# uibk-uncover/ws-unet

Hardware: AMD Instinct MI355X
Metric: 512x512 grayscale images/sec (UNet predict) (higher is better)
Workload: dtype f16 MFMA on the f16 halves + ONE block-scaled fp4 (e2m1) MFMA per tap pair for both residual cross terms (per-pixel / per-(co, tap) E8M0 scales), fp32 accumulate; planar storage

## Files before the change

### ws_unet_amd/csrc/conv3x3_q.hip

```cpp
#include "wsu_device.h"
#include <cstdlib>

#ifndef WSU_Q_EPO
#define WSU_Q_EPO 1
#endif
#ifndef WSU_Q_PIPE2
#define WSU_Q_PIPE2 0
#endif
#ifndef WSU_Q_PIPE_DEPTH
#define WSU_Q_PIPE_DEPTH 1
#endif
#ifndef WSU_Q_PROBE_NOX8
#define WSU_Q_PROBE_NOX8 0
#endif
#ifndef WSU_Q_EPO_FENCE
#define WSU_Q_EPO_FENCE 1
#endif

namespace {

constexpr int TW = 32, TH = 16, IW = TW + 2, IH = TH + 2;
constexpr int NPIX = IW * IH;
constexpr int PLANE = NPIX * 16;
constexpr int IN_SEG = (NPIX + 63) / 64;
constexpr int S_LDS = IN_SEG * 256;
constexpr int IN_SLOT = 3 * PLANE + S_LDS;
constexpr int W_GRAN = 9 * 3 * WSU_COB * 16;
constexpr int W_SLOT = W_GRAN + 1024;
constexpr int NIN = 3, NWS = 2;
constexpr int W_BASE = NIN * IN_SLOT;
constexpr int LDS_EXTRA = W_BASE + NWS * W_SLOT;
constexpr int LDS_TOTAL = LDS_EXTRA + 1024 * 4 + 4 * 64 * 4 + 16;
static_assert(LDS_TOTAL <= 160 * 1024 && W_SLOT % 1024 == 0, "LDS budget");
constexpr int NLOAD = 4;
constexpr int W_PIECES = W_SLOT / 1024;
constexpr unsigned OOB = 0xFFFFFFF0u;
constexpr int IN_SLOT_H = 2 * PLANE;
constexpr int W_SLOT_H = 9 * 2 * WSU_COB * 16;
template <int FMT> struct QGeo {
    static_assert(FMT == WSU_PLANAR_Q || FMT == WSU_PLANAR_H, "conv3x3_q_kernel formats: Q and H");
    static constexpr bool H = FMT == WSU_PLANAR_H;
    static constexpr int in_slot = H ? IN_SLOT_H : IN_SLOT, w_slot = H ? W_SLOT_H : W_SLOT;
    static constexpr int w_planes = H ? 2 : 3;
    static constexpr int w_base = NIN * in_slot, lds_extra = w_base + NWS * w_slot;
    static constexpr int lds_total = lds_extra + 1024 * 4 + 4 * 64 * 4 + 16;
    static constexpr int w_pieces = w_slot / 1024;
};
static_assert(QGeo<WSU_PLANAR_Q>::lds_total == LDS_TOTAL && QGeo<WSU_PLANAR_Q>::w_pieces == W_PIECES && W_SLOT_H % 1024 == 0, "LDS geometry");

struct QArgs {
    const char* x1; const char* x2; const char* wp; const float* bias;
    char* y; char* ypool;
    const float* head_w; const float* head_b; float* head_out; float* head_logit; int head_cout;
    int n, h, w, c1, c2, cout;
    int tiles_x, tiles_y, ncb, nch1, nch;
    int relu;
    int ntiles;
    unsigned* range_flag;
    int msplit;
    int ablate;
    const float* img; const float* w1; const float* b1;
};

struct Tile { int n, y0, x0, cb, mh; };
__device__ __forceinline__ Tile tile_of(const QArgs& a, int t) {
    Tile r;
    r.cb = t % a.ncb; t /= a.ncb;
    const int tx = t % a.tiles_x; t /= a.tiles_x;
    const int ty = t % a.tiles_y;
    r.n = t / a.tiles_y; r.y0 = ty * TH; r.x0 = tx * TW;
    r.mh = 0;
    if (a.msplit) { r.mh = r.cb & 1; r.cb >>= 1; }
    return r;
}

typedef __attribute__((address_space(3))) void lds_void;
typedef __attribute__((address_space(3))) char lds_char;

__device__ __forceinline__ float dpp_xor1(float v) {
    return __builtin_bit_cast(float, __builtin_amdgcn_update_dpp(0, __builtin_bit_cast(int, v), 0xB1 , 0xF, 0xF, true));
}

template <int FMT, int LW>
__device__ __forceinline__ void q_loader(const QArgs& a, char* smem, int lane, int lw, int G, int J) {
    using Gm = QGeo<FMT>;
    constexpr int NSEG = LW < 2 ? 3 : 2;
    constexpr int NIN_OPS = (Gm::H ? 2 : 4) * NSEG;
    constexpr int W0 = Gm::H ? (LW < 2 ? LW * 3 : 6 + (LW - 2) * 6) : (LW < 2 ? LW * 5 : 10 + (LW - 2) * 9);
    constexpr int NWP = Gm::H ? (LW < 2 ? 3 : 6) : (LW < 2 ? 5 : 9);
    static_assert(2 * 5 + 2 * 9 == W_PIECES && 2 * 3 + 2 * 6 == QGeo<WSU_PLANAR_H>::w_pieces, "weight pieces over the loader waves");
    lds_char* smem3 = (lds_char*)smem;
    const unsigned hw16 = (unsigned)(a.h * a.w) * 16u;
    const unsigned chunk_bytes = Gm::H ? (unsigned)wsu_h_chunk_bytes(a.h, a.w) : (unsigned)wsu_q_chunk_bytes(a.h, a.w);
    unsigned voff[NSEG], soff[NSEG];
    auto plan = [&](const Tile& t) __attribute__((always_inline)) {
        WSU_STATIC_FOR(NSEG, k, {
            const int idx = min((LW + NLOAD * k) * 64 + lane, NPIX - 1);
            const int r = idx / IW, c = idx - r * IW;
            const int yy = wsu_reflect(t.y0 - 1 + r, a.h), xx = wsu_reflect(t.x0 - 1 + c, a.w);
            voff[k] = (unsigned)(yy * a.w + xx) * 16u;
            if constexpr (!Gm::H) soff[k] = 3u * hw16 + wsu_q_soff(yy, xx, a.tiles_x);
        });
    };
    Tile ti = tile_of(a, lw); int ci = 0, kti = 0;
    int cbw = ti.cb, cw = 0, ktw = 0;
    auto issue_in = [&](int s) __attribute__((always_inline)) {
        const char* in_src = ci < a.nch1 ? a.x1 + ((size_t)ti.n * a.nch1 + ci) * chunk_bytes : a.x2 + ((size_t)ti.n * (a.nch - a.nch1) + (ci - a.nch1)) * chunk_bytes;
        const auto rs_in = __builtin_amdgcn_make_buffer_rsrc(const_cast<char*>(in_src), 0, (int)chunk_bytes, 0x00020000);
        lds_char* slot = smem3 + (s % NIN) * Gm::in_slot;
        WSU_STATIC_FOR(NSEG, k, {
            constexpr int seg = LW + NLOAD * k;
            const bool live = seg < IN_SEG - 1 || lane < NPIX - (IN_SEG - 1) * 64;
            if (live) {
                __builtin_amdgcn_raw_ptr_buffer_load_lds(rs_in, (lds_void*)(slot + seg * 1024), 16, voff[k], 0, 0, 0);
                __builtin_amdgcn_raw_ptr_buffer_load_lds(rs_in, (lds_void*)(slot + PLANE + seg * 1024), 16, voff[k], (int)hw16, 0, 0);
                if constexpr (!Gm::H) {
                    __builtin_amdgcn_raw_ptr_buffer_load_lds(rs_in, (lds_void*)(slot + 2 * PLANE + seg * 1024), 16, voff[k], (int)(2u * hw16), 0, 0);
                    __builtin_amdgcn_raw_ptr_buffer_load_lds(rs_in, (lds_void*)(slot + 3 * PLANE + seg * 256), 1, soff[k], 0, 0, 0);
                }
            }
        });
        if (++ci == a.nch && s + 1 < J) { ci = 0; ++kti; ti = tile_of(a, lw + kti * G); plan(ti); }
    };
    auto issue_w = [&](int s) __attribute__((always_inline)) {
        const auto rs_w = __builtin_amdgcn_make_buffer_rsrc(const_cast<char*>(a.wp), 0, 0x7FFFFFF0, 0x00020000);
        const int w_base = (cbw * a.nch + cw) * Gm::w_slot;
        lds_char* slot = smem3 + Gm::w_base + (s % NWS) * Gm::w_slot;
        WSU_STATIC_FOR(NWP, k, {
            constexpr int piece = W0 + k;
            __builtin_amdgcn_raw_ptr_buffer_load_lds(rs_w, (lds_void*)(slot + piece * 1024), 16, (unsigned)lane * 16u, w_base + piece * 1024, 0, 0);
        });
        if (++cw == a.nch && s + 1 < J) { cw = 0; ++ktw; cbw = tile_of(a, lw + ktw * G).cb; }
    };
    if (J <= 0) return;
    plan(ti);
    issue_w(0);
    issue_in(0);
    if (J > 1) issue_in(1);
    if (J > 1) asm volatile("s_waitcnt vmcnt(%0)" :: "n"(NIN_OPS) : "memory"); else asm volatile("s_waitcnt vmcnt(0)" ::: "memory");
    for (int j = 0; ; ++j) {
        __builtin_amdgcn_s_barrier();
        asm volatile("" ::: "memory");
        if (j + 1 >= J) break;
        if (!(a.ablate & 1)) {
            issue_w(j + 1);
            const bool more = j + 2 < J;
            if (more) issue_in(j + 2);
            if (more) asm volatile("s_waitcnt vmcnt(%0)" :: "n"(NIN_OPS) : "memory"); else asm volatile("s_waitcnt vmcnt(0)" ::: "memory");
        }
    }
}

__device__ __forceinline__ void q_loader_f1(const QArgs& a, char* smem, int lane, int lw, int G, int J, int lw8) {
    if (J <= 0) return;
    if (a.ablate & 16) __builtin_amdgcn_s_setprio(3);
    lds_char* smem3 = (lds_char*)smem;
    constexpr int F1_PX = 3;
    float pimg[F1_PX][9];
    float f1_max = 0.f;
    Tile ti = tile_of(a, lw); int ci = 0, kti = 0;
    int cbw = ti.cb, cw = 0, ktw = 0;
    auto window = [&](const Tile& tt) __attribute__((always_inline)) {
        const float* img = a.img + (size_t)tt.n * a.h * a.w;
#pragma unroll
        for (int k = 0; k < F1_PX; ++k) {
            const int idx = min((lw8 + NLOAD * k) * 64 + lane, NPIX - 1);
            const int r = idx / IW, cc = idx - r * IW;
            const int yy = wsu_reflect(tt.y0 - 1 + r, a.h), xx = wsu_reflect(tt.x0 - 1 + cc, a.w);
#pragma unroll
            for (int tp = 0; tp < 9; ++tp)
                pimg[k][tp] = img[(size_t)wsu_reflect(yy + tp / 3 - 1, a.h) * a.w + wsu_reflect(xx + tp % 3 - 1, a.w)];
        }
    };
    typedef __attribute__((address_space(4))) const f32x2 cst_f32x2;
    auto compute_in = [&](int s) __attribute__((always_inline)) {
        char* slot = smem + (s % NIN) * IN_SLOT;
        cst_f32x2* wt = (cst_f32x2*)(a.w1 + ci * 16);
        cst_f32x2* bt = (cst_f32x2*)(a.b1 + ci * 16);
        f32x2 acc[F1_PX][8];
#pragma unroll
        for (int g = 0; g < 8; ++g) {
            const f32x2 b = bt[g];
#pragma unroll
            for (int k = 0; k < F1_PX; ++k) acc[k][g] = b;
        }
#pragma unroll
        for (int tp = 0; tp < 9; ++tp) {
            f32x2 wv[8];
#pragma unroll
            for (int g = 0; g < 8; ++g) wv[g] = wt[tp * 32 + g];
#pragma unroll
            for (int k = 0; k < F1_PX; ++k) {
                const f32x2 pw = {pimg[k][tp & ~1], pimg[k][(tp | 1) < 9 ? (tp | 1) : tp]};
#pragma unroll
                for (int g = 0; g < 8; ++g) {
                    if (tp & 1) asm volatile("v_pk_fma_f32 %0, %1, %2, %0 op_sel:[1,0,0] op_sel_hi:[1,1,1]" : "+v"(acc[k][g]) : "v"(pw), "s"(wv[g]));
                    else asm volatile("v_pk_fma_f32 %0, %1, %2, %0 op_sel:[0,0,0] op_sel_hi:[0,1,1]" : "+v"(acc[k][g]) : "v"(pw), "s"(wv[g]));
                }
            }
        }
        asm volatile("s_nop 0" ::: "memory");
#pragma unroll
        for (int k = 0; k < F1_PX; ++k) {
            const int idx = (lw8 + NLOAD * k) * 64 + lane;
            f32x4 v[4];
#pragma unroll
            for (int g = 0; g < 4; ++g) v[g] = mk_f4(acc[k][2 * g][0], acc[k][2 * g][1], acc[k][2 * g + 1][0], acc[k][2 * g + 1][1]);
#pragma unroll
            for (int g = 0; g < 4; ++g)
#pragma unroll
                for (int e = 0; e < 4; ++e) { v[g][e] = fmaxf(v[g][e], 0.f); f1_max = fmaxf(f1_max, v[g][e]); }
            u32x4 h0, h1, qg; uint32_t sb;
            wsu_q4_encode16(v, h0, h1, qg, sb);
            if (lw8 + NLOAD * k < IN_SEG && idx < NPIX) {
                char* d = slot + idx * 16;
                *reinterpret_cast<u32x4*>(d) = h0;
                *reinterpret_cast<u32x4*>(d + PLANE) = h1;
                *reinterpret_cast<u32x4*>(d + 2 * PLANE) = qg;
                *reinterpret_cast<uint32_t*>(slot + 3 * PLANE + idx * 4) = sb;
            }
        }
        if (++ci == a.nch && s + 1 < J) { ci = 0; ++kti; ti = tile_of(a, lw + kti * G); window(ti); }
    };
    const int w0 = lw8 < 2 ? lw8 * 5 : 10 + (lw8 - 2) * 9, nwp = lw8 < 2 ? 5 : 9;
    auto issue_w = [&](int s) __attribute__((always_inline)) {
        const auto rs_w = __builtin_amdgcn_make_buffer_rsrc(const_cast<char*>(a.wp), 0, 0x7FFFFFF0, 0x00020000);
        const int w_base = (cbw * a.nch + cw) * W_SLOT;
        lds_char* slot = smem3 + W_BASE + (s % NWS) * W_SLOT;
#pragma unroll
        for (int k = 0; k < 9; ++k)
            if (k < nwp)
                __builtin_amdgcn_raw_ptr_buffer_load_lds(rs_w, (lds_void*)(slot + (w0 + k) * 1024), 16, (unsigned)lane * 16u, w_base + (w0 + k) * 1024, 0, 0);
        if (++cw == a.nch && s + 1 < J) { cw = 0; ++ktw; cbw = tile_of(a, lw + ktw * G).cb; }
    };
    window(ti);
    issue_w(0);
    compute_in(0);
    if (J > 1) compute_in(1);
    asm volatile("s_waitcnt vmcnt(0) lgkmcnt(0)" ::: "memory");
    for (int j = 0; ; ++j) {
        __builtin_amdgcn_s_barrier();
        asm volatile("" ::: "memory");
        if (j + 1 >= J) break;
        issue_w(j + 1);
        if (j + 2 < J) compute_in(j + 2);
        asm volatile("s_waitcnt vmcnt(0) lgkmcnt(0)" ::: "memory");
    }
    if (a.range_flag && __builtin_amdgcn_ballot_w64(!(f1_max <= WSU_F8_RANGE)) != 0 && lane == 0) atomicOr(a.range_flag, 1u);
}

template <int RQ, int HC, bool POOL, bool FQ, bool MSPLIT, bool F1 = false, int FMT = WSU_PLANAR_Q>
__global__ __launch_bounds__((16 / RQ + NLOAD) * 64) __attribute__((amdgpu_waves_per_eu(RQ == 4 ? 2 : 3, RQ == 4 ? 2 : 3)))
void conv3x3_q_kernel(const QArgs a) {
    using Gm = QGeo<FMT>;
    constexpr bool H = Gm::H;
    static_assert(!(H && F1), "the fused first layer computes Q inputs");
    constexpr int NWAVE = 16 / RQ, NT = (NWAVE + NLOAD) * 64;
    extern __shared__ __attribute__((aligned(16))) char smem[];
    const int tid = threadIdx.x;
    const int wv = __builtin_amdgcn_readfirstlane(tid >> 6), lane = tid & 63, l31 = lane & 31, hh = lane >> 5;
    const int l31_k = l31, hh_k = hh;
    const int G = gridDim.x;
    const int lw = (int)wsu_xcd_remap(blockIdx.x, G);
    const int K = a.ntiles > lw ? (a.ntiles - lw + G - 1) / G : 0;
    const int J = K * a.nch;

    float* s_bias = reinterpret_cast<float*>(smem + Gm::lds_extra);
    float* s_hw = s_bias + 1024;
    float* s_hb = s_hw + 4 * 64;
    for (int i = tid; i < a.cout; i += NT) s_bias[i] = a.bias ? a.bias[i] : 0.f;
    constexpr bool HEAD = HC > 0;
    if constexpr (HEAD) {
        for (int i = tid; i < a.head_cout * 64; i += NT) s_hw[i] = a.head_w[i];
        if (tid < 4) s_hb[tid] = (a.head_b && tid < a.head_cout) ? a.head_b[tid] : 0.f;
    }

    if (wv >= NWAVE) {
        if constexpr (F1) { q_loader_f1(a, smem, lane, lw, G, J, wv - NWAVE); return; }
        switch (wv - NWAVE) {
            case 0: q_loader<FMT, 0>(a, smem, lane, lw, G, J); break;
            case 1: q_loader<FMT, 1>(a, smem, lane, lw, G, J); break;
            case 2: q_loader<FMT, 2>(a, smem, lane, lw, G, J); break;
            default: q_loader<FMT, 3>(a, smem, lane, lw, G, J); break;
        }
        return;
    }

    Tile cur = tile_of(a, lw);
    constexpr int MH = MSPLIT ? 1 : 2;
    constexpr bool PIPE = (RQ == 4 || WSU_Q_PIPE2) && !H;
    constexpr bool EPO = WSU_Q_EPO && !MSPLIT && HC == 0 && RQ != 4;
    f32x16 acc[2][4];
    int kt = 0, j = 0;
    unsigned q_in_off = 0, q_w_off = 0;
    const char* ldsA = smem;
    const char* ldsB = smem;
    int hh_q = hh;
    auto begin_step = [&]() __attribute__((always_inline)) {
        __builtin_amdgcn_s_barrier();
        asm volatile("" ::: "memory");
        q_in_off = (unsigned)(j % NIN) * Gm::in_slot; q_w_off = Gm::w_base + (unsigned)(j % NWS) * Gm::w_slot;
        ldsA = smem + q_w_off + (cur.mh * 32 + l31) * 16;
        ldsB = smem + q_in_off + ((RQ * wv) * IW + l31) * 16;
        hh_q = hh;
        asm volatile("" : "+v"(hh_q));
    };
    auto zero_acc = [&]() __attribute__((always_inline)) {
#pragma unroll
        for (int m = 0; m < MH; ++m)
#pragma unroll
            for (int q = 0; q < RQ; ++q)
#pragma unroll
                for (int r = 0; r < 16; ++r) acc[m][q][r] = 0.f;
    };
    auto main_term = [&](auto tap_c, auto ms_c) __attribute__((always_inline)) {
        constexpr int tap = decltype(tap_c)::value, dy = tap / 3, dx = tap % 3;
        constexpr int ms = decltype(ms_c)::value, ML = ms < 0 ? 0 : ms, MU = ms < 0 ? MH : ms + 1;
        u32x4 ah[2], bh[4];
_Pragma("unroll")
        for (int m = ML; m < MU; ++m) ah[m] = *reinterpret_cast<const u32x4*>(ldsA + ((tap * Gm::w_planes + hh) * 64 + m * 32) * 16);
_Pragma("unroll")
        for (int q = 0; q < RQ; ++q) bh[q] = *reinterpret_cast<const u32x4*>(ldsB + hh * PLANE + ((q + dy) * IW + dx) * 16);
_Pragma("unroll")
        for (int m = ML; m < MU; ++m)
_Pragma("unroll")
            for (int q = 0; q < RQ; ++q) wsu_mfma_f16(ah[m], bh[q], acc[m][q]);
    };
    auto cross_q4 = [&](auto tp_c, auto ms_c) __attribute__((always_inline)) {
        constexpr int tp = decltype(tp_c)::value;
        constexpr int ms = decltype(ms_c)::value, ML = ms < 0 ? 0 : ms, MU = ms < 0 ? MH : ms + 1;
        constexpr int t0 = 2 * tp, t1 = (2 * tp + 1 < 9) ? 2 * tp + 1 : 2 * tp;
        constexpr bool single = 2 * tp + 1 >= 9;
        const int tap = hh_q ? t1 : t0;
        const int pixoff = (tap / 3) * IW + tap % 3;
        u32x4 a4[2], b4[4]; int sa[2], sb[4];
        typedef __attribute__((address_space(3))) const unsigned char lds_cuchar;
        typedef __attribute__((address_space(3))) const int lds_cint;
        typedef __attribute__((address_space(3))) const u32x4 lds_cu32x4;
        lds_char* L = (lds_char*)smem;
        const unsigned wbase = q_w_off + (unsigned)(cur.mh * 32 + l31) * 16u + (unsigned)((tap * 3 + 2) * 64) * 16u;
        const unsigned sabase = q_w_off + W_GRAN + (unsigned)(tap * 64 + cur.mh * 32 + l31);
        const unsigned pix = (unsigned)((RQ * wv) * IW + l31 + pixoff);
_Pragma("unroll")
        for (int m = ML; m < MU; ++m) {
            a4[m] = *(lds_cu32x4*)(L + wbase + m * 32 * 16);
            sa[m] = *(lds_cuchar*)(L + sabase + m * 32);
        }
_Pragma("unroll")
        for (int q = 0; q < RQ; ++q) {
            b4[q] = *(lds_cu32x4*)(L + q_in_off + 2 * PLANE + (pix + q * IW) * 16u);
            sb[q] = *(lds_cint*)(L + q_in_off + 3 * PLANE + (pix + q * IW) * 4u);
        }
        if (single && hh_q) {
            const u32x4 z = mk_u4(0, 0, 0, 0);
_Pragma("unroll")
            for (int m = ML; m < MU; ++m) a4[m] = z;
_Pragma("unroll")
            for (int q = 0; q < RQ; ++q) b4[q] = z;
        }
_Pragma("unroll")
        for (int m = ML; m < MU; ++m)
_Pragma("unroll")
            for (int q = 0; q < RQ; ++q) wsu_mfma_q4(a4[m], b4[q], sa[m], sb[q], acc[m][q]);
    };
    auto units_range = [&](auto ms_c, auto lo_c, auto hi_c) __attribute__((always_inline)) {
        constexpr int lo = decltype(lo_c)::value, hi = decltype(hi_c)::value;
        if constexpr (EPO) asm volatile("" : "+v"(hh_q));
        WSU_STATIC_FOR(hi - lo, i, {
            constexpr int tp = lo + i;
            if constexpr (!H && !(WSU_Q_PROBE_NOX8 && tp == 4)) cross_q4(std::integral_constant<int, tp>{}, ms_c);
            main_term(std::integral_constant<int, 2 * tp>{}, ms_c);
            if constexpr (2 * tp + 1 < 9) main_term(std::integral_constant<int, 2 * tp + 1>{}, ms_c);
        });
    };
    constexpr std::integral_constant<int, -1> all_m{};
    struct Frag { u32x4 a[2]; u32x4 b[4]; int sa[2]; int sb[4]; };
    auto load_unit = [&](auto u_c, Frag& f) __attribute__((always_inline)) {
        constexpr int u = decltype(u_c)::value, tp = u / 3, k = u % 3;
        typedef __attribute__((address_space(3))) const unsigned char lds_cuchar;
        typedef __attribute__((address_space(3))) const int lds_cint;
        typedef __attribute__((address_space(3))) const u32x4 lds_cu32x4;
        lds_char* L = (lds_char*)smem;
        if constexpr (k == 0) {
            constexpr int t0 = 2 * tp, t1 = (2 * tp + 1 < 9) ? 2 * tp + 1 : 2 * tp;
            const int tap = hh_q ? t1 : t0;
            const int pixoff = (tap / 3) * IW + tap % 3;
            const unsigned wbase = q_w_off + (unsigned)(cur.mh * 32 + l31) * 16u + (unsigned)((tap * 3 + 2) * 64) * 16u;
            const unsigned sabase = q_w_off + W_GRAN + (unsigned)(tap * 64 + cur.mh * 32 + l31);
            const unsigned pix = (unsigned)((RQ * wv) * IW + l31 + pixoff);
_Pragma("unroll")
            for (int m = 0; m < MH; ++m) {
                f.a[m] = *(lds_cu32x4*)(L + wbase + m * 32 * 16);
                f.sa[m] = *(lds_cuchar*)(L + sabase + m * 32);
            }
_Pragma("unroll")
            for (int q = 0; q < RQ; ++q) {
                f.b[q] = *(lds_cu32x4*)(L + q_in_off + 2 * PLANE + (pix + q * IW) * 16u);
                f.sb[q] = *(lds_cint*)(L + q_in_off + 3 * PLANE + (pix + q * IW) * 4u);
            }
        } else {
            constexpr int tap = 2 * tp + k - 1, dy = tap / 3, dx = tap % 3;
            const unsigned abase = q_w_off + (unsigned)((cur.mh * 32 + l31) * 16) + (unsigned)(hh_q * 64 * 16);
            const unsigned bbase = q_in_off + (unsigned)(((RQ * wv) * IW + l31) * 16) + (unsigned)(hh_q * PLANE);
_Pragma("unroll")
            for (int m = 0; m < MH; ++m) f.a[m] = *(lds_cu32x4*)(L + abase + ((tap * 3) * 64 + m * 32) * 16);
_Pragma("unroll")
            for (int q = 0; q < RQ; ++q) f.b[q] = *(lds_cu32x4*)(L + bbase + ((q + dy) * IW + dx) * 16);
        }
    };
    auto mma_unit = [&](auto u_c, Frag& f) __attribute__((always_inline)) {
        constexpr int u = decltype(u_c)::value, tp = u / 3, k = u % 3;
        if constexpr (k == 0) {
            if (2 * tp + 1 >= 9 && hh_q) {
                const u32x4 z = mk_u4(0, 0, 0, 0);
_Pragma("unroll")
                for (int m = 0; m < MH; ++m) f.a[m] = z;
_Pragma("unroll")
                for (int q = 0; q < RQ; ++q) f.b[q] = z;
            }
_Pragma("unroll")
            for (int m = 0; m < MH; ++m)
_Pragma("unroll")
                for (int q = 0; q < RQ; ++q) wsu_mfma_q4(f.a[m], f.b[q], f.sa[m], f.sb[q], acc[m][q]);
        } else {
_Pragma("unroll")
            for (int m = 0; m < MH; ++m)
_Pragma("unroll")
                for (int q = 0; q < RQ; ++q) wsu_mfma_f16(f.a[m], f.b[q], acc[m][q]);
        }
    };
    auto units_pipelined = [&]() __attribute__((always_inline)) {
        constexpr int NU = 14, D = WSU_Q_PIPE_DEPTH, NS = D + 1;
        Frag fr[NS];
        WSU_STATIC_FOR(D, u, { load_unit(u_c, fr[u % NS]); });
        WSU_STATIC_FOR(NU, u, {
            if constexpr (u + D < NU) load_unit(std::integral_constant<int, u + D>{}, fr[(u + D) % NS]);
            __builtin_amdgcn_sched_barrier(0);
            mma_unit(u_c, fr[u % NS]);
            __builtin_amdgcn_sched_barrier(0);
        });
    };
    auto units_all = [&](auto ms_c) __attribute__((always_inline)) {
        if constexpr (PIPE && decltype(ms_c)::value < 0) { units_pipelined(); return; }
        units_range(ms_c, std::integral_constant<int, 0>{}, std::integral_constant<int, 5>{});
    };

    auto finish_tile = [&]() __attribute__((always_inline)) {
        int l31 = l31_k, hh = hh_k;
        asm volatile("" : "+v"(l31), "+v"(hh));
        const int col = cur.x0 + l31;
        const unsigned hw16 = (unsigned)(a.h * a.w) * 16u;
        const int nco = a.cout >> 4;
        float hz[4][HC > 0 ? HC : 1];
        float vmax = 0.f;
        const float relu_floor = a.relu ? 0.f : -__builtin_inff();
#pragma unroll
        for (int q = 0; q < RQ; ++q)
#pragma unroll
            for (int o = 0; o < (HC > 0 ? HC : 1); ++o) hz[q][o] = 0.f;
        auto store_pair_q = [&](const f32x4& X0, const f32x4& Y0, const f32x4& X1, const f32x4& Y1, char* base, unsigned chunk_bytes, unsigned plane_bytes,
                                unsigned off0, unsigned off1, unsigned soff0, unsigned soff1, bool ok0, bool ok1, bool have) __attribute__((always_inline)) {
            u32x4 g0, g1; uint32_t dh0, dr0, sb0, dh1, dr1, sb1;
            wsu_q4_pre(X0, Y0, g0, dh0, dr0, sb0);
            wsu_q4_pre(X1, Y1, g1, dh1, dr1, sb1);
            const u32x4 qg = wsu_q4_pair(dh0, dr0, dh1, dr1);
            const auto rs = __builtin_amdgcn_make_buffer_rsrc(base, 0, have ? (int)chunk_bytes : 0, 0x00020000);
            const unsigned hp = hh ? plane_bytes : 0u;
            __builtin_amdgcn_raw_buffer_store_b128(g0, rs, (int)(ok0 ? off0 + hp : OOB), 0, 0);
            __builtin_amdgcn_raw_buffer_store_b128(g1, rs, (int)(ok1 ? off1 + hp : OOB), 0, 0);
            const bool okm = hh ? ok1 : ok0;
            __builtin_amdgcn_raw_buffer_store_b128(qg, rs, (int)(okm ? (hh ? off1 : off0) + 2u * plane_bytes : OOB), 0, 0);
            __builtin_amdgcn_raw_buffer_store_b8((unsigned char)(hh ? sb1 : sb0), rs, (int)(okm ? 3u * plane_bytes + (hh ? soff1 : soff0) : OOB), 0, 0);
        };
        auto store_one_q = [&](const f32x4& X, const f32x4& Y, char* base, unsigned chunk_bytes, unsigned plane_bytes, unsigned off, unsigned soff, bool ok, bool have) __attribute__((always_inline)) {
            u32x4 g; uint32_t dh, dr, sb;
            wsu_q4_pre(X, Y, g, dh, dr, sb);
            const u32x4 qg = wsu_q4_single(dh, dr);
            const auto rs = __builtin_amdgcn_make_buffer_rsrc(base, 0, have ? (int)chunk_bytes : 0, 0x00020000);
            __builtin_amdgcn_raw_buffer_store_b128(g, rs, (int)(ok ? off + (hh ? plane_bytes : 0u) : OOB), 0, 0);
            __builtin_amdgcn_raw_buffer_store_b128(qg, rs, (int)((ok && !hh) ? off + 2u * plane_bytes : OOB), 0, 0);
            __builtin_amdgcn_raw_buffer_store_b8((unsigned char)sb, rs, (int)((ok && !hh) ? 3u * plane_bytes + soff : OOB), 0, 0);
        };
        auto store_one_h = [&](const f32x4& X, const f32x4& Y, char* base, unsigned plane_bytes, unsigned off, bool ok, bool have) __attribute__((always_inline)) {
            const auto rs = __builtin_amdgcn_make_buffer_rsrc(base, 0, have ? (int)(2u * plane_bytes) : 0, 0x00020000);
            __builtin_amdgcn_raw_buffer_store_b128(wsu_h_granule(X, Y), rs, (int)(ok ? off + (hh ? plane_bytes : 0u) : OOB), 0, 0);
        };
        auto store_one_a = [&](const f32x4& X, const f32x4& Y, char* base, unsigned plane_bytes, unsigned off, bool ok, bool have) __attribute__((always_inline)) {
            uint32_t xh0, xh1, xlo, yh0, yh1, ylo;
            wsu_split4_f16r8(X, WSU_F8_XLO_DIV, xh0, xh1, xlo);
            wsu_split4_f16r8(Y, WSU_F8_XLO_DIV, yh0, yh1, ylo);
            wsu_swap32(xh0, yh0); wsu_swap32(xh1, yh1);
            uint32_t xlp = xlo, ylp = ylo;
            wsu_swap32(xlo, xlp); wsu_swap32(ylo, ylp);
            const auto rs = __builtin_amdgcn_make_buffer_rsrc(base, 0, have ? (int)(3u * plane_bytes) : 0, 0x00020000);
            __builtin_amdgcn_raw_buffer_store_b128(mk_u4(xh0, xh1, yh0, yh1), rs, (int)(ok ? off + (hh ? plane_bytes : 0u) : OOB), 0, 0);
            __builtin_amdgcn_raw_buffer_store_b128(mk_u4(xlo, xlp, ylo, ylp), rs, (int)((ok && !hh) ? off + 2u * plane_bytes : OOB), 0, 0);
        };
        auto epi_m = [&](auto m_c, auto&& hook) __attribute__((always_inline)) {
            constexpr int m = decltype(m_c)::value;
            constexpr int NH = RQ / 2;
            auto piece = [&](auto cp_c) __attribute__((always_inline)) {
                constexpr int cp = decltype(cp_c)::value;
                const int oc = cur.cb * 4 + (m + cur.mh) * 2 + cp;
                const int co0 = oc * 16 + 4 * hh;
                const bool have_y = a.y != nullptr;
                f32x4 px[2], py[2];
                WSU_STATIC_FOR(RQ / 2, rp, {
                    hook(std::integral_constant<int, NH * cp + rp>{});
                    f32x4 vx[2], vy[2];
                    const f32x4 bx = *reinterpret_cast<const f32x4*>(s_bias + co0), by = *reinterpret_cast<const f32x4*>(s_bias + co0 + 8);
_Pragma("unroll")
                    for (int u = 0; u < 2; ++u) {
_Pragma("unroll")
                        for (int e = 0; e < 4; ++e) {
                            const float x = fmaxf(acc[m][2 * rp + u][8 * cp + e] + bx[e], relu_floor), y = fmaxf(acc[m][2 * rp + u][8 * cp + 4 + e] + by[e], relu_floor);
                            vx[u][e] = x; vy[u][e] = y;
                            vmax = fmaxf(vmax, fmaxf(fabsf(x), fabsf(y)));
                        }
                    }
                    if constexpr (HEAD) {
                        const int lc = (m * 2 + cp) * 16 + 4 * hh;
_Pragma("unroll")
                        for (int o = 0; o < HC; ++o)
// ... 26 lines not shown
                            });
                        }
                    }
                    if constexpr (POOL) {
_Pragma("unroll")
                        for (int e = 0; e < 4; ++e) {
                            const float cx = fmaxf(vx[0][e], vx[1][e]), cy = fmaxf(vy[0][e], vy[1][e]);
                            px[rp][e] = fmaxf(cx, dpp_xor1(cx)); py[rp][e] = fmaxf(cy, dpp_xor1(cy));
                        }
                    }
                });
                if constexpr (POOL) {
                    const int hp = a.h >> 1, wp2 = a.w >> 1;
                    const int gy0 = (cur.y0 >> 1) + (RQ / 2) * wv, gx = (cur.x0 >> 1) + (l31 >> 1);
                    const bool okx = !(l31 & 1) && gx < wp2;
                    const unsigned php16 = (unsigned)(hp * wp2) * 16u;
                    if constexpr (H) {
                        char* base = a.ypool + ((size_t)cur.n * nco + oc) * (2u * php16);
#pragma unroll
                        for (int rp = 0; rp < RQ / 2; ++rp)
                            store_one_h(px[rp], py[rp], base, php16, (unsigned)((gy0 + rp) * wp2 + gx) * 16u, okx && gy0 + rp < hp, true);
                    } else if constexpr (FQ) {
                        const unsigned cbp = (unsigned)wsu_q_chunk_bytes(hp, wp2);
                        const int ptx = (wp2 + 31) >> 5;
                        char* base = a.ypool + ((size_t)cur.n * nco + oc) * cbp;
                        if constexpr (RQ == 4) {
                            store_pair_q(px[0], py[0], px[1], py[1], base, cbp, php16, (unsigned)(gy0 * wp2 + gx) * 16u, (unsigned)((gy0 + 1) * wp2 + gx) * 16u,
                                         wsu_q_soff(gy0, gx, ptx), wsu_q_soff(gy0 + 1, gx, ptx), okx && gy0 < hp, okx && gy0 + 1 < hp, true);
                        } else {
                            store_one_q(px[0], py[0], base, cbp, php16, (unsigned)(gy0 * wp2 + gx) * 16u, wsu_q_soff(gy0, gx, ptx), okx && gy0 < hp, true);
                        }
                    } else {
                        char* base = a.ypool + (((size_t)cur.n * nco + oc) * 3) * php16;
#pragma unroll
                        for (int rp = 0; rp < RQ / 2; ++rp)
                            store_one_a(px[rp], py[rp], base, php16, (unsigned)((gy0 + rp) * wp2 + gx) * 16u, okx && gy0 + rp < hp, true);
                    }
                }
            };
            piece(std::integral_constant<int, 0>{});
            piece(std::integral_constant<int, 1>{});
        };
        auto nothing = [](auto) __attribute__((always_inline)) {};
        if constexpr (EPO) {
            constexpr int NHT = 2 * (RQ / 2);
            epi_m(std::integral_constant<int, 0>{}, [&](auto h_c) __attribute__((always_inline)) {
                constexpr int h = decltype(h_c)::value;
                constexpr int lo = 5 * h / NHT, hi = 5 * (h + 1) / NHT;
                if constexpr (WSU_Q_EPO_FENCE && RQ == 4) __builtin_amdgcn_sched_barrier(0);
                if constexpr (hi > lo) units_range(std::integral_constant<int, 1>{}, std::integral_constant<int, lo>{}, std::integral_constant<int, hi>{});
            });
            if constexpr (WSU_Q_EPO_FENCE && RQ == 4) __builtin_amdgcn_sched_barrier(0);
            epi_m(std::integral_constant<int, 1>{}, nothing);
        } else {
            WSU_STATIC_FOR(MH, m, { (void)m; epi_m(m_c, nothing); });
        }
        if constexpr (HEAD) {
            const size_t hw = (size_t)a.h * a.w;
#pragma unroll
            for (int q = 0; q < RQ; ++q) {
                const int row = cur.y0 + RQ * wv + q;
#pragma unroll
                for (int o = 0; o < HC; ++o)
                    if (o < a.head_cout) {
                        uint32_t mine = __builtin_bit_cast(uint32_t, hz[q][o]), other = mine;
                        wsu_swap32(mine, other);
                        const float z = __builtin_bit_cast(float, mine) + __builtin_bit_cast(float, other) + s_hb[o];
                        if (!hh && row < a.h && col < a.w) {
                            const size_t plane = ((size_t)cur.n * a.head_cout + o) * hw;
                            const uint32_t off = (uint32_t)(row * a.w + col);
                            if (a.head_logit) (a.head_logit + plane)[off] = z;
                            (a.head_out + plane)[off] = 1.f / (1.f + expf(-z));
                        }
                    }
            }
        }
        if (a.range_flag && (a.y || POOL) && __builtin_amdgcn_ballot_w64(!(vmax <= (H ? WSU_F16_RANGE : WSU_F8_RANGE))) != 0 && lane == 0)
            atomicOr(a.range_flag, 1u);
        ++kt;
        if (j + 1 < J) cur = tile_of(a, lw + kt * G);
    };
    for (int t = 0; t < K; ++t) {
        zero_acc();
        for (int cc = 1; cc < a.nch; ++cc) { begin_step(); units_all(all_m); ++j; }
        begin_step();
        if constexpr (EPO) units_all(std::integral_constant<int, 0>{});
        else units_all(all_m);
        if (a.ablate & 2) {
            if constexpr (EPO) units_all(std::integral_constant<int, 1>{});
#pragma unroll
            for (int m = 0; m < MH; ++m)
#pragma unroll
                for (int q = 0; q < RQ; ++q) asm volatile("" :: "v"(acc[m][q]));
            ++kt;
            if (j + 1 < J) cur = tile_of(a, lw + kt * G);
        } else {
            finish_tile();
        }
        ++j;
    }
}

__global__ void pack_conv3x3_f4_kernel(const float* __restrict__ w, char* __restrict__ dst, int cin, int cout) {
    const int nch = cin / 16;
    const long long total = (long long)(cout / WSU_COB) * nch * 9 * WSU_COB;
    for (long long d = (long long)blockIdx.x * blockDim.x + threadIdx.x; d < total; d += (long long)gridDim.x * blockDim.x) {
        long long t = d;
        const int co = (int)(t % WSU_COB); t /= WSU_COB;
        const int tap = (int)(t % 9); t /= 9;
        const int c = (int)(t % nch); const int cb = (int)(t / nch);
        float v[16], r[16];
        uint32_t h[8];
#pragma unroll
        for (int e = 0; e < 16; ++e) v[e] = w[(((size_t)(cb * WSU_COB + co) * cin + c * 16 + e) * 3 + tap / 3) * 3 + tap % 3];
#pragma unroll
        for (int e = 0; e < 8; ++e) {
            const _Float16 a = (_Float16)v[2 * e], b = (_Float16)v[2 * e + 1];
            h[e] = (uint32_t)__builtin_bit_cast(unsigned short, a) | ((uint32_t)__builtin_bit_cast(unsigned short, b) << 16);
            r[2 * e] = (v[2 * e] - (float)a) * 2048.f; r[2 * e + 1] = (v[2 * e + 1] - (float)b) * 2048.f;
        }
        const u32x4 h0 = mk_u4(h[0], h[1], h[2], h[3]), h1 = mk_u4(h[4], h[5], h[6], h[7]);
        const int E = wsu_q4_block_exp(wsu_f16x16_max_abs_bits(h0, h1));
        const float sc = wsu_pow2f(E);
        uint32_t q[4] = {0, 0, 0, 0};
        WSU_STATIC_FOR(8, e, { q[e >> 2] = __builtin_amdgcn_cvt_scalef32_pk_fp4_f32(q[e >> 2], r[2 * e], r[2 * e + 1], sc, e & 3); });
        q[2] = wsu_f16x8_to_fp4(h0, sc); q[3] = wsu_f16x8_to_fp4(h1, sc);
        char* slice = dst + ((size_t)cb * nch + c) * W_SLOT;
        char* base = slice + (size_t)(tap * 3) * (WSU_COB * 16) + co * 16;
        *reinterpret_cast<u32x4*>(base) = h0;
        *reinterpret_cast<u32x4*>(base + WSU_COB * 16) = h1;
        *reinterpret_cast<u32x4*>(base + 2 * WSU_COB * 16) = mk_u4(q[0], q[1], q[2], q[3]);
        slice[W_GRAN + tap * 64 + co] = (char)(E + 127 - 11);
        if (tap == 0 && co < 7) *reinterpret_cast<u32x4*>(slice + W_GRAN + 576 + co * 64) = mk_u4(0, 0, 0, 0), *reinterpret_cast<u32x4*>(slice + W_GRAN + 576 + co * 64 + 16) = mk_u4(0, 0, 0, 0),
            *reinterpret_cast<u32x4*>(slice + W_GRAN + 576 + co * 64 + 32) = mk_u4(0, 0, 0, 0), *reinterpret_cast<u32x4*>(slice + W_GRAN + 576 + co * 64 + 48) = mk_u4(0, 0, 0, 0);
    }
}

__global__ void pack_conv3x3_h_kernel(const float* __restrict__ w, char* __restrict__ dst, int cin, int cout) {
    const int nch = cin / 16;
    const long long total = (long long)(cout / WSU_COB) * nch * 9 * WSU_COB;
    for (long long d = (long long)blockIdx.x * blockDim.x + threadIdx.x; d < total; d += (long long)gridDim.x * blockDim.x) {
        long long t = d;
        const int co = (int)(t % WSU_COB); t /= WSU_COB;
        const int tap = (int)(t % 9); t /= 9;
        const int c = (int)(t % nch); const int cb = (int)(t / nch);
        uint32_t h[8];
#pragma unroll
        for (int e = 0; e < 8; ++e) {
            const size_t i0 = (((size_t)(cb * WSU_COB + co) * cin + c * 16 + 2 * e) * 3 + tap / 3) * 3 + tap % 3;
            const _Float16 a = (_Float16)w[i0], b = (_Float16)w[i0 + 9];
            h[e] = (uint32_t)__builtin_bit_cast(unsigned short, a) | ((uint32_t)__builtin_bit_cast(unsigned short, b) << 16);
        }
        char* base = dst + ((size_t)cb * nch + c) * W_SLOT_H + (size_t)(tap * 2) * (WSU_COB * 16) + co * 16;
        *reinterpret_cast<u32x4*>(base) = mk_u4(h[0], h[1], h[2], h[3]);
        *reinterpret_cast<u32x4*>(base + WSU_COB * 16) = mk_u4(h[4], h[5], h[6], h[7]);
    }
}

#define WSU_Q_INST(RQ) \
    template __global__ void conv3x3_q_kernel<RQ, 0, false, false, false>(const QArgs); \
    template __global__ void conv3x3_q_kernel<RQ, 0, false, true, false>(const QArgs);  \
    template __global__ void conv3x3_q_kernel<RQ, 0, true, false, false>(const QArgs);  \
    template __global__ void conv3x3_q_kernel<RQ, 0, true, true, false>(const QArgs);   \
    template __global__ void conv3x3_q_kernel<RQ, 1, false, false, false>(const QArgs); \
    template __global__ void conv3x3_q_kernel<RQ, 4, false, false, false>(const QArgs); \
    template __global__ void conv3x3_q_kernel<RQ, 0, false, false, true>(const QArgs);  \
    template __global__ void conv3x3_q_kernel<RQ, 0, false, true, true>(const QArgs);
WSU_Q_INST(4)
WSU_Q_INST(2)
template __global__ void conv3x3_q_kernel<2, 0, true, true, false, true>(const QArgs);
template __global__ void conv3x3_q_kernel<2, 0, false, true, false, false, WSU_PLANAR_H>(const QArgs);
template __global__ void conv3x3_q_kernel<2, 0, true, true, false, false, WSU_PLANAR_H>(const QArgs);
template __global__ void conv3x3_q_kernel<2, 1, false, true, false, false, WSU_PLANAR_H>(const QArgs);
template __global__ void conv3x3_q_kernel<2, 4, false, true, false, false, WSU_PLANAR_H>(const QArgs);
template __global__ void conv3x3_q_kernel<2, 0, false, true, true, false, WSU_PLANAR_H>(const QArgs);

template <int RQ>
int q_launch_rq(QArgs a, int yq, hipStream_t s, int ncu, bool msplit_on) {
    constexpr int NT = (16 / RQ + NLOAD) * 64;
    static bool attr_done = false;
    if (!attr_done) {
        const void* fns[8] = {reinterpret_cast<const void*>(&conv3x3_q_kernel<RQ, 0, false, false, false>), reinterpret_cast<const void*>(&conv3x3_q_kernel<RQ, 0, false, true, false>),
                              reinterpret_cast<const void*>(&conv3x3_q_kernel<RQ, 0, true, false, false>), reinterpret_cast<const void*>(&conv3x3_q_kernel<RQ, 0, true, true, false>),
                              reinterpret_cast<const void*>(&conv3x3_q_kernel<RQ, 1, false, false, false>), reinterpret_cast<const void*>(&conv3x3_q_kernel<RQ, 4, false, false, false>),
                              reinterpret_cast<const void*>(&conv3x3_q_kernel<RQ, 0, false, false, true>), reinterpret_cast<const void*>(&conv3x3_q_kernel<RQ, 0, false, true, true>)};
        for (const void* fn : fns) {
            hipError_t e = hipFuncSetAttribute(fn, hipFuncAttributeMaxDynamicSharedMemorySize, LDS_TOTAL);
            if (e != hipSuccess) { wsu_set_error("hipFuncSetAttribute(conv3x3_q): %s", hipGetErrorString(e)); return WSU_ERR_HIP; }
        }
        attr_done = true;
    }
    a.msplit = 0;
    if (msplit_on && !a.head_w && !a.ypool && 2 * (long long)a.ntiles <= ncu) {
        a.msplit = 1; a.ncb *= 2; a.ntiles *= 2;
        if (yq) hipLaunchKernelGGL((conv3x3_q_kernel<RQ, 0, false, true, true>), dim3(a.ntiles), dim3(NT), LDS_TOTAL, s, a);
        else hipLaunchKernelGGL((conv3x3_q_kernel<RQ, 0, false, false, true>), dim3(a.ntiles), dim3(NT), LDS_TOTAL, s, a);
        return wsu_check_launch("conv3x3_q_kernel<msplit>");
    }
    const dim3 g(a.ntiles < ncu ? a.ntiles : ncu), b(NT);
    if (a.head_w && a.head_cout == 1) hipLaunchKernelGGL((conv3x3_q_kernel<RQ, 1, false, false, false>), g, b, LDS_TOTAL, s, a);
    else if (a.head_w) hipLaunchKernelGGL((conv3x3_q_kernel<RQ, 4, false, false, false>), g, b, LDS_TOTAL, s, a);
    else if (a.ypool && yq) hipLaunchKernelGGL((conv3x3_q_kernel<RQ, 0, true, true, false>), g, b, LDS_TOTAL, s, a);
    else if (a.ypool) hipLaunchKernelGGL((conv3x3_q_kernel<RQ, 0, true, false, false>), g, b, LDS_TOTAL, s, a);
    else if (yq) hipLaunchKernelGGL((conv3x3_q_kernel<RQ, 0, false, true, false>), g, b, LDS_TOTAL, s, a);
    else hipLaunchKernelGGL((conv3x3_q_kernel<RQ, 0, false, false, false>), g, b, LDS_TOTAL, s, a);
    return wsu_check_launch("conv3x3_q_kernel");
}

int h_launch(QArgs a, hipStream_t s, int ncu, bool msplit_on) {
    constexpr int HF = WSU_PLANAR_H, NT = (8 + NLOAD) * 64, LDS = QGeo<HF>::lds_total;
    static bool attr_done = false;
    if (!attr_done) {
        const void* fns[5] = {reinterpret_cast<const void*>(&conv3x3_q_kernel<2, 0, false, true, false, false, HF>),
                              reinterpret_cast<const void*>(&conv3x3_q_kernel<2, 0, true, true, false, false, HF>),
                              reinterpret_cast<const void*>(&conv3x3_q_kernel<2, 1, false, true, false, false, HF>),
                              reinterpret_cast<const void*>(&conv3x3_q_kernel<2, 4, false, true, false, false, HF>),
                              reinterpret_cast<const void*>(&conv3x3_q_kernel<2, 0, false, true, true, false, HF>)};
        for (const void* fn : fns) {
            hipError_t e = hipFuncSetAttribute(fn, hipFuncAttributeMaxDynamicSharedMemorySize, LDS);
            if (e != hipSuccess) { wsu_set_error("hipFuncSetAttribute(conv3x3_q<H>): %s", hipGetErrorString(e)); return WSU_ERR_HIP; }
        }
        attr_done = true;
    }
    a.msplit = 0;
    if (msplit_on && !a.head_w && !a.ypool && 2 * (long long)a.ntiles <= ncu) {
        a.msplit = 1; a.ncb *= 2; a.ntiles *= 2;
        hipLaunchKernelGGL((conv3x3_q_kernel<2, 0, false, true, true, false, HF>), dim3(a.ntiles), dim3(NT), LDS, s, a);
        return wsu_check_launch("conv3x3_q_kernel<H, msplit>");
    }
    const dim3 g(a.ntiles < ncu ? a.ntiles : ncu), b(NT);
    if (a.head_w && a.head_cout == 1) hipLaunchKernelGGL((conv3x3_q_kernel<2, 1, false, true, false, false, HF>), g, b, LDS, s, a);
    else if (a.head_w) hipLaunchKernelGGL((conv3x3_q_kernel<2, 4, false, true, false, false, HF>), g, b, LDS, s, a);
    else if (a.ypool) hipLaunchKernelGGL((conv3x3_q_kernel<2, 0, true, true, false, false, HF>), g, b, LDS, s, a);
    else hipLaunchKernelGGL((conv3x3_q_kernel<2, 0, false, true, false, false, HF>), g, b, LDS, s, a);
    return wsu_check_launch("conv3x3_q_kernel<H>");
}

}

extern "C" {

size_t wsu_conv3x3_packed_f4_bytes(int cin, int cout) {
    if (cin <= 0 || cout <= 0 || cin % 16 || cout % WSU_COB) return 0;
    return (size_t)(cout / WSU_COB) * (cin / 16) * W_SLOT;
}
int wsu_conv3x3_pack_f4(const float* w_oihw, void* w_packed, int cin, int cout, void* stream) {
    WSU_REQUIRE(w_oihw && w_packed, "conv3x3_pack_f4: null pointer");
    WSU_REQUIRE(cin > 0 && cin % 16 == 0 && cout > 0 && cout % WSU_COB == 0, "conv3x3_pack_f4: cin=%d must be a multiple of 16, cout=%d of %d", cin, cout, WSU_COB);
    hipLaunchKernelGGL(pack_conv3x3_f4_kernel, dim3(512), dim3(256), 0, static_cast<hipStream_t>(stream), w_oihw, (char*)w_packed, cin, cout);
    return wsu_check_launch("pack_conv3x3_f4_kernel");
}

int wsu_conv3x3_q_fused_first_fwd(const float* img, const float* w1_taps, const float* b1, const void* w_packed_f4, const float* bias, void* y, void* y_pool,
                                  int n, int h, int w, int cout, int relu, unsigned* range_flag, void* stream) {
    const float* w1 = w1_taps;
    WSU_REQUIRE(img && w1 && b1 && w_packed_f4 && y && y_pool, "conv3x3_q_fused_first: null pointer");
    WSU_REQUIRE(((uintptr_t)w1 & 63) == 0 && ((uintptr_t)b1 & 63) == 0, "conv3x3_q_fused_first: w1_taps and b1 must be 64-byte aligned (scalar 16-dword loads)");
    WSU_REQUIRE(n > 0 && h >= 2 && w >= 2 && h % 2 == 0 && w % 2 == 0, "conv3x3_q_fused_first: bad shape n=%d h=%d w=%d (even h, w: the pooled output)", n, h, w);
    WSU_REQUIRE(cout > 0 && cout % WSU_COB == 0 && cout <= 1024, "conv3x3_q_fused_first: cout=%d must be a multiple of %d (<= 1024)", cout, WSU_COB);
    WSU_REQUIRE((long long)h * w * 50 < 0xFFFFFFF0LL, "conv3x3_q_fused_first: h*w too large (a chunk must stay below 4 GiB)");
    QArgs a;
    a.x1 = nullptr; a.x2 = nullptr; a.wp = (const char*)w_packed_f4; a.bias = bias;
    a.y = (char*)y; a.ypool = (char*)y_pool;
    a.head_w = nullptr; a.head_b = nullptr; a.head_out = nullptr; a.head_logit = nullptr; a.head_cout = 0;
    a.range_flag = range_flag;
    a.n = n; a.h = h; a.w = w; a.c1 = 64; a.c2 = 0; a.cout = cout;
    a.tiles_x = (w + TW - 1) / TW; a.tiles_y = (h + TH - 1) / TH; a.ncb = cout / WSU_COB;
    static int prio = -1;
    if (prio < 0) { const char* e = getenv("WSU_Q_F1_PRIO"); prio = (e && atoi(e)) ? 1 : 0; }
    a.nch1 = 4; a.nch = 4; a.relu = relu; a.msplit = 0; a.ablate = prio ? 16 : 0;
    a.img = img; a.w1 = w1; a.b1 = b1;
    const long long nt = (long long)n * a.tiles_x * a.tiles_y * a.ncb;
    WSU_REQUIRE(nt > 0 && nt < 0x3FFFFFFFLL, "conv3x3_q_fused_first: %lld tiles out of range", nt);
    a.ntiles = (int)nt;
    static int ncu = 0;
    if (ncu == 0) {
        int dev = 0; hipDeviceProp_t prop;
        if (hipGetDevice(&dev) != hipSuccess || hipGetDeviceProperties(&prop, dev) != hipSuccess) {
            wsu_set_error("conv3x3_q_fused_first: cannot query the device"); return WSU_ERR_HIP;
        }
        hipError_t e = hipFuncSetAttribute(reinterpret_cast<const void*>(&conv3x3_q_kernel<2, 0, true, true, false, true>), hipFuncAttributeMaxDynamicSharedMemorySize, LDS_TOTAL);
        if (e != hipSuccess) { wsu_set_error("hipFuncSetAttribute(conv3x3_q<F1>): %s", hipGetErrorString(e)); return WSU_ERR_HIP; }
        ncu = prop.multiProcessorCount;
    }
    hipLaunchKernelGGL((conv3x3_q_kernel<2, 0, true, true, false, true>), dim3(a.ntiles < ncu ? a.ntiles : ncu), dim3((8 + NLOAD) * 64), LDS_TOTAL,
                       static_cast<hipStream_t>(stream), a);
    return wsu_check_launch("conv3x3_q_kernel<F1>");
}

size_t wsu_planar_q_bytes(int n, int c, int h, int w) {
    if (n <= 0 || c <= 0 || c % 16 || h <= 0 || w <= 0) return 0;
    return (size_t)n * (size_t)(c / 16) * wsu_q_chunk_bytes(h, w);
}

int wsu_conv3x3_q_fwd(const void* x1, const void* x2, const void* w_packed_f4, const float* bias, void* y, void* y_pool,
                      const float* head_w, const float* head_b, float* head_out, float* head_logit, int head_cout,
                      int n, int h, int w, int c1, int c2, int cout, int relu, int y_format, unsigned* range_flag, void* stream) {
    WSU_REQUIRE(x1 && w_packed_f4 && (y || y_pool || head_w), "conv3x3_q: null pointer");
    WSU_REQUIRE(n > 0 && h >= 2 && w >= 2, "conv3x3_q: bad shape n=%d h=%d w=%d (reflect pad 1 needs h,w >= 2)", n, h, w);
    WSU_REQUIRE(c1 > 0 && c1 % 16 == 0 && c2 >= 0 && c2 % 16 == 0 && (c2 == 0) == (x2 == nullptr), "conv3x3_q: c1=%d c2=%d must be multiples of 16", c1, c2);
    WSU_REQUIRE(cout > 0 && cout % WSU_COB == 0 && cout <= 1024, "conv3x3_q: cout=%d must be a multiple of %d (<= 1024)", cout, WSU_COB);
    WSU_REQUIRE(!head_w || (head_out && cout == WSU_COB && head_cout >= 1 && head_cout <= 4), "conv3x3_q: fused head needs cout == %d and 1..4 head planes", WSU_COB);
    WSU_REQUIRE(!y_pool || (h % 2 == 0 && w % 2 == 0), "conv3x3_q: fused pool needs even h, w");
    WSU_REQUIRE(!(y_pool && head_w), "conv3x3_q: the fused pool and the fused head exclude each other");
    WSU_REQUIRE(y_format == WSU_PLANAR_A || y_format == WSU_PLANAR_Q, "conv3x3_q: y_format must be WSU_PLANAR_A or WSU_PLANAR_Q");
    WSU_REQUIRE(!(head_w && y && y_format != WSU_PLANAR_A), "conv3x3_q: a y beside the fused head is written in format WSU_PLANAR_A");
    WSU_REQUIRE((long long)h * w * 50 < 0xFFFFFFF0LL, "conv3x3_q: h*w too large (a chunk must stay below 4 GiB)");
    QArgs a;
    a.x1 = (const char*)x1; a.x2 = (const char*)x2; a.wp = (const char*)w_packed_f4; a.bias = bias;
    a.y = (char*)y; a.ypool = (char*)y_pool;
    a.head_w = head_w; a.head_b = head_b; a.head_out = head_out; a.head_logit = head_logit; a.head_cout = head_cout;
    a.range_flag = range_flag;
    a.n = n; a.h = h; a.w = w; a.c1 = c1; a.c2 = c2; a.cout = cout;
    a.tiles_x = (w + TW - 1) / TW; a.tiles_y = (h + TH - 1) / TH; a.ncb = cout / WSU_COB;
    a.nch1 = c1 / 16; a.nch = (c1 + c2) / 16; a.relu = relu;
    a.img = nullptr; a.w1 = nullptr; a.b1 = nullptr;
    const long long nt = (long long)n * a.tiles_x * a.tiles_y * a.ncb;
    WSU_REQUIRE(nt > 0 && nt < 0x3FFFFFFFLL, "conv3x3_q: %lld tiles out of range", nt);
    a.ntiles = (int)nt;
    static int ncu = 0, rq = 0, msplit_on = 1, ablate = 0;
    if (ncu == 0) {
        int dev = 0; hipDeviceProp_t prop;
        if (hipGetDevice(&dev) != hipSuccess || hipGetDeviceProperties(&prop, dev) != hipSuccess) {
// ... 68 lines not shown
```

Before: 3635.

## Defer last tap's f16 MFMA across the barrier and add timing stamps

For the non-pipelined f16 path, the tap-8 operands are loaded from LDS before the step ends, and their MFMA runs after the next barrier. This overlaps the LDS read latency with barrier wait, at the cost of extra registers to hold the deferred operands. It also adds an explicit lgkmcnt(0) wait before every compute-wave barrier. That wait may add stalls. Optional s_memtime stamp instrumentation is added under WSU_Q_STAMPS and is off by default.

```diff
diff --git a/ws_unet_amd/csrc/conv3x3_q.hip b/ws_unet_amd/csrc/conv3x3_q.hip
--- a/ws_unet_amd/csrc/conv3x3_q.hip
+++ b/ws_unet_amd/csrc/conv3x3_q.hip
@@ -77,6 +77,20 @@
 typedef __attribute__((address_space(3))) void lds_void;
 typedef __attribute__((address_space(3))) char lds_char;
 
+#ifdef WSU_Q_STAMPS
+constexpr int Q_NW = 12, Q_NST = 10;
+__device__ unsigned long long g_q_stamps[256 * Q_NW * Q_NST];
+#define Q_STAMP(v) v = __builtin_amdgcn_s_memtime()
+__device__ __forceinline__ void q_stamps_store(int wv, const unsigned long long (&v)[Q_NST]) {
+    if (blockIdx.x >= 256 || wv >= Q_NW || (threadIdx.x & 63)) return;
+    unsigned long long* d = g_q_stamps + (blockIdx.x * Q_NW + wv) * Q_NST;
+    for (int i = 0; i < Q_NST; ++i) d[i] = v[i];
+}
+#define Q_SIMD_ID() ((unsigned long long)__builtin_amdgcn_s_getreg(4 | (4 << 6) | (1 << 11)))
+#else
+#define Q_STAMP(v) do {} while (0)
+#endif
+
 __device__ __forceinline__ float dpp_xor1(float v) {
     return __builtin_bit_cast(float, __builtin_amdgcn_update_dpp(0, __builtin_bit_cast(int, v), 0xB1 , 0xF, 0xF, true));
 }
@@ -138,17 +152,36 @@
     issue_in(0);
     if (J > 1) issue_in(1);
     if (J > 1) asm volatile("s_waitcnt vmcnt(%0)" :: "n"(NIN_OPS) : "memory"); else asm volatile("s_waitcnt vmcnt(0)" ::: "memory");
+#ifdef WSU_Q_STAMPS
+    unsigned long long st[Q_NST] = {}, st_a, st_b, st_c;
+    st[0] = Q_SIMD_ID(); st[2] = (unsigned long long)J;
+    const unsigned long long st_t0 = __builtin_amdgcn_s_memtime(), st_rt0 = __builtin_amdgcn_s_memrealtime();
+#endif
     for (int j = 0; ; ++j) {
+        Q_STAMP(st_a);
         __builtin_amdgcn_s_barrier();
         asm volatile("" ::: "memory");
+        Q_STAMP(st_b);
+#ifdef WSU_Q_STAMPS
+        st[4] += st_b - st_a;
+#endif
         if (j + 1 >= J) break;
         if (!(a.ablate & 1)) {
             issue_w(j + 1);
             const bool more = j + 2 < J;
             if (more) issue_in(j + 2);
+            Q_STAMP(st_c);
             if (more) asm volatile("s_waitcnt vmcnt(%0)" :: "n"(NIN_OPS) : "memory"); else asm volatile("s_waitcnt vmcnt(0)" ::: "memory");
-        }
-    }
+#ifdef WSU_Q_STAMPS
+            Q_STAMP(st_a);
+            st[1] += st_c - st_b; st[3] += st_a - st_c;
+#endif
+        }
+    }
+#ifdef WSU_Q_STAMPS
+    st[8] = __builtin_amdgcn_s_memtime() - st_t0; st[9] = __builtin_amdgcn_s_memrealtime() - st_rt0;
+    q_stamps_store(8 + LW, st);
+#endif
 }
 
 __device__ __forceinline__ void q_loader_f1(const QArgs& a, char* smem, int lane, int lw, int G, int J, int lw8) {
@@ -287,6 +320,12 @@
     }
 
     Tile cur = tile_of(a, lw);
+#ifdef WSU_Q_STAMPS
+    unsigned long long st[Q_NST] = {}, st_a = 0, st_rel = 0, st_b = 0;
+    bool st_open = true;
+    st[0] = Q_SIMD_ID();
+    const unsigned long long st_t0 = __builtin_amdgcn_s_memtime(), st_rt0 = __builtin_amdgcn_s_memrealtime();
+#endif
     constexpr int MH = MSPLIT ? 1 : 2;
     constexpr bool PIPE = (RQ == 4 || WSU_Q_PIPE2) && !H;
     constexpr bool EPO = WSU_Q_EPO && !MSPLIT && HC == 0 && RQ != 4;
@@ -297,8 +336,16 @@
     const char* ldsB = smem;
     int hh_q = hh;
     auto begin_step = [&]() __attribute__((always_inline)) {
+        Q_STAMP(st_a);
+        asm volatile("s_waitcnt lgkmcnt(0)" ::: "memory");
         __builtin_amdgcn_s_barrier();
         asm volatile("" ::: "memory");
+#ifdef WSU_Q_STAMPS
+        Q_STAMP(st_b);
+        if (st_open) st[4] += st_b - st_a;
+        else { st[1] += st_a - st_rel; ++st[2]; st[3] += st_b - st_a; }
+        st_open = false; st_rel = st_b;
+#endif
         q_in_off = (unsigned)(j % NIN) * Gm::in_slot; q_w_off = Gm::w_base + (unsigned)(j % NWS) * Gm::w_slot;
         ldsA = smem + q_w_off + (cur.mh * 32 + l31) * 16;
         ldsB = smem + q_in_off + ((RQ * wv) * IW + l31) * 16;
@@ -351,6 +398,12 @@
             b4[q] = *(lds_cu32x4*)(L + q_in_off + 2 * PLANE + (pix + q * IW) * 16u);
             sb[q] = *(lds_cint*)(L + q_in_off + 3 * PLANE + (pix + q * IW) * 4u);
         }
+#ifdef WSU_Q_STAMPS
+        if constexpr (tp == 0 && ms <= 0) {
+            asm volatile("s_waitcnt lgkmcnt(0)" ::: "memory");
+            unsigned long long st_f; Q_STAMP(st_f); st[5] += st_f - st_rel;
+        }
+#endif
         if (single && hh_q) {
             const u32x4 z = mk_u4(0, 0, 0, 0);
 _Pragma("unroll")
@@ -439,6 +492,29 @@
             mma_unit(u_c, fr[u % NS]);
             __builtin_amdgcn_sched_barrier(0);
         });
+    };
+    constexpr bool DEFER = !PIPE && !H;
+    u32x4 dfa[2], dfb[4];
+    auto defer_zero = [&]() __attribute__((always_inline)) {
+_Pragma("unroll")
+        for (int m = 0; m < MH; ++m) dfa[m] = mk_u4(0, 0, 0, 0);
+_Pragma("unroll")
+        for (int q = 0; q < RQ; ++q) dfb[q] = mk_u4(0, 0, 0, 0);
+    };
+    auto defer_mma = [&]() __attribute__((always_inline)) {
+_Pragma("unroll")
+        for (int m = 0; m < MH; ++m)
+_Pragma("unroll")
+            for (int q = 0; q < RQ; ++q) wsu_mfma_f16(dfa[m], dfb[q], acc[m][q]);
+    };
+    auto units_deferring = [&]() __attribute__((always_inline)) {
+        units_range(all_m, std::integral_constant<int, 0>{}, std::integral_constant<int, 4>{});
+        cross_q4(std::integral_constant<int, 4>{}, all_m);
+        constexpr int tap = 8, dy = tap / 3, dx = tap % 3;
+_Pragma("unroll")
+        for (int m = 0; m < MH; ++m) dfa[m] = *reinterpret_cast<const u32x4*>(ldsA + ((tap * Gm::w_planes + hh) * 64 + m * 32) * 16);
+_Pragma("unroll")
+        for (int q = 0; q < RQ; ++q) dfb[q] = *reinterpret_cast<const u32x4*>(ldsB + hh * PLANE + ((q + dy) * IW + dx) * 16);
     };
     auto units_all = [&](auto ms_c) __attribute__((always_inline)) {
         if constexpr (PIPE && decltype(ms_c)::value < 0) { units_pipelined(); return; }
@@ -631,8 +707,15 @@
     };
     for (int t = 0; t < K; ++t) {
         zero_acc();
-        for (int cc = 1; cc < a.nch; ++cc) { begin_step(); units_all(all_m); ++j; }
-        begin_step();
+        if constexpr (DEFER) {
+            defer_zero();
+            for (int cc = 1; cc < a.nch; ++cc) { begin_step(); defer_mma(); units_deferring(); ++j; }
+            begin_step();
+            defer_mma();
+        } else {
+            for (int cc = 1; cc < a.nch; ++cc) { begin_step(); units_all(all_m); ++j; }
+            begin_step();
+        }
         if constexpr (EPO) units_all(std::integral_constant<int, 0>{});
         else units_all(all_m);
         if (a.ablate & 2) {
@@ -644,10 +727,21 @@
             ++kt;
             if (j + 1 < J) cur = tile_of(a, lw + kt * G);
         } else {
+            Q_STAMP(st_b);
             finish_tile();
+#ifdef WSU_Q_STAMPS
+            Q_STAMP(st_a); st[6] += st_a - st_b; ++st[7];
+#endif
         }
         ++j;
-    }
+#ifdef WSU_Q_STAMPS
+        st_open = true;
+#endif
+    }
+#ifdef WSU_Q_STAMPS
+    st[8] = __builtin_amdgcn_s_memtime() - st_t0; st[9] = __builtin_amdgcn_s_memrealtime() - st_rt0;
+    q_stamps_store(wv, st);
+#endif
 }
 
 __global__ void pack_conv3x3_f4_kernel(const float* __restrict__ w, char* __restrict__ dst, int cin, int cout) {
@@ -788,6 +882,13 @@
 }
 
 extern "C" {
+
+#ifdef WSU_Q_STAMPS
+int wsu_debug_read_q_stamps(unsigned long long* host_dst, int nblocks) {
+    if (nblocks > 256) nblocks = 256;
+    return hipMemcpyFromSymbol(host_dst, HIP_SYMBOL(g_q_stamps), sizeof(unsigned long long) * Q_NW * Q_NST * nblocks, 0, hipMemcpyDeviceToHost) == hipSuccess ? 0 : 1;
+}
+#endif
 
 size_t wsu_conv3x3_packed_f4_bytes(int cin, int cout) {
     if (cin <= 0 || cout <= 0 || cin % 16 || cout % WSU_COB) return 0;
```

Result: no change. 3668, median of 6 (+0.9%).
